# shanice-l/UNOPose

Hardware: AMD Instinct MI355X
Metric: (query,ref) pairs/sec forward (higher is better)
Workload: dtype bf16; 1 GPU; UNOPose.forward, batch 32 pairs/GPU, 2048 query pts, 5000->2048 reference pts, 196 coarse pts, 518x518 crops, DINOv2 ViT-B/14 reg4, random-init (trained-like) weights

## Files before the change

include/unopose_hip.h:

```cpp
#ifndef UNOPOSE_HIP_H
#define UNOPOSE_HIP_H

#include <stdint.h>

#ifdef __cplusplus
extern "C" {
#endif

#define UNOPOSE_OK 0
#define UNOPOSE_EINVAL 1
#define UNOPOSE_ELAUNCH 2
#define UNOPOSE_ENOMEM 3

typedef void *unopose_stream_t;

int unopose_abi_version(void);
const char *unopose_last_error(void);


int unopose_furthest_point_sampling(const float *xyz, int B, int N, int M,
                                    int32_t *idx, unopose_stream_t stream);

int unopose_gather_points(const float *points, const int32_t *idx, int B, int C,
                          int N, int M, float *out, unopose_stream_t stream);
// ... 110 lines not shown
int unopose_conv1x1_train_wgrad_blocks(void);
int unopose_conv1x1_train_forward(const float *x, int B, int cin, long L, const float *w, int cout, float *y, unopose_stream_t stream);
int unopose_conv1x1_train_wgrad(const float *dy, const float *x, int B, int cout, int cin, long L, float *workspace, float *dw,
                                unopose_stream_t stream);

int unopose_linear_wgrad_f32_splits(long rows, int N, int K);
int unopose_linear_wgrad_f32(const float *g, const float *x, long rows, int N, int K, float *workspace, float *dw, unopose_stream_t stream);

int unopose_linear_small_train_ws_floats(long rows, int N, int K);
int unopose_linear_small_train_forward(const float *x, const float *w, const float *bias, long rows, int N, int K, int relu, float *y,
                                       unopose_stream_t stream);
int unopose_linear_small_train_dx(const float *g, const float *y, const float *w, long rows, int N, int K, float *dx, unopose_stream_t stream);
int unopose_linear_small_train_dwdb(const float *g, const float *y, const float *x, long rows, int N, int K, float *workspace, long workspace_floats,
                                    float *dw, float *db, unopose_stream_t stream);
int unopose_linear_small_train_backward(const float *g, const float *y, const float *x, const float *w, long rows, int N, int K, float *workspace,
                                        long workspace_floats, float *dx, float *dw, float *db, unopose_stream_t stream);
int unopose_assign_labels(const float *atten, int B, int R, int C, const float *score1,
                          const float *score2, float *stats_ws, float *w1, float *w2,
                          unopose_stream_t stream);

int unopose_fine_correspondences(const float *atten, int B, int R, int C, const float *score1,
                                 const float *score2, const float *stats_ws, const float *w1,
                                 const float *w2, const float *pts2, float *weight, float *pred,
                                 unopose_stream_t stream);

int unopose_upproj_plan(const long long *choose, int B2, int Np, int H, int W, int side, int tok_offset, int tok_stride,
                        int cap_rows, int *ws, int *row_list, int *cellmap, int *tile_info, unopose_stream_t stream);

int unopose_linear_bf16_ld(const void *A, int lda, const void *W, int ldw, const float *bias, void *C, int ldc, long M, int N, int K,
                           int epilogue, unopose_stream_t stream);

int unopose_linear_add_layernorm_bf16(const void *A, const void *W, const float *bias, const void *resid, const float *ln_w,
                                      const float *ln_b, float eps, void *C, long M, int K, unopose_stream_t stream);

int unopose_linear_bf16_kv_vt(const void *A, const void *W, const float *bias, void *C, void *vt, long M, int N, int K, int tokens, int key_pad,
                              unopose_stream_t stream);

int unopose_linear_bf16_gather(const void *A, long M, int K, const void *W, int N, const float *bias, const int *row_list,
                               const int *tile_info, int max_tiles, void *C, unopose_stream_t stream);

int unopose_bilinear_sample_compact(const void *Cc, const int *cellmap, const long long *choose, int B2, int side, int Np,
                                    int H, int W, void *out, int out_bf16, unopose_stream_t stream);

int unopose_fine_assign(const void *f1, const void *f2, int B, int R, int C, int D, float shift, const float *score1,
                        const float *score2, const float *pts2, float *ws, float *w1, float *w2, float *weight,
                        float *pred, unopose_stream_t stream);

int unopose_min_dist(const float *p, const float *q, int B, int N, int M, const float *R,
                     const float *t, int cand_per_b, float *out, unopose_stream_t stream);

int unopose_coarse_hypotheses(const float *atten, int B, int R, int C, const float *score1,
                              const float *score2, const float *stats_ws, const float *w1,
                              const float *w2, const float *rand, int nprop, const float *pts1,
                              const float *pts2, float *cdf_ws, float *Rout, float *tout,
                              float *dis, unopose_stream_t stream);

int unopose_coarse_scores(const float *pts1, const float *pts2, int B, int n1, int n2,
                          const float *Rall, const float *tall, int nprop, const int64_t *top,
                          int ncand, const float *w1, float *score, unopose_stream_t stream);

int unopose_topk_smallest(const float *x, int B, int n, int k, int64_t *idx, unopose_stream_t stream);
int unopose_coarse_pick(const float *score, const int64_t *top, int B, int ncand, const float *Rall, const float *tall, int nprop,
                        float *R, float *t, float *best_score, unopose_stream_t stream);

int unopose_token_attention(const void *q, int ldq, const void *k, int ldk, const void *vt,
                            const void *qp, int ldqp, const void *E, int B, int n, int m,
// ... 215 lines not shown
```

unopose_amd/_lib.py:

```python
import ctypes
import os

import torch

_HERE = os.path.dirname(os.path.abspath(__file__))
SO_PATH = os.environ.get("UNOPOSE_LIB") or os.path.join(_HERE, "libunopose_hip.so")

_lib = None

_P = ctypes.c_void_p
_I = ctypes.c_int
_F = ctypes.c_float
_L = ctypes.c_long
_D = ctypes.c_double

SIGNATURES = {
    "unopose_furthest_point_sampling": [_P, _I, _I, _I, _P, _P],
    "unopose_gather_points": [_P, _P, _I, _I, _I, _I, _P, _P],
    "unopose_gather_points_grad": [_P, _P, _I, _I, _I, _I, _P, _P],
    "unopose_ball_query": [_P, _P, _I, _I, _I, _F, _I, _P, _P],
    "unopose_group_points": [_P, _P, _I, _I, _I, _I, _I, _P, _P],
    "unopose_group_points_grad": [_P, _P, _I, _I, _I, _I, _I, _P, _P],
    "unopose_three_nn": [_P, _P, _I, _I, _I, _P, _P, _P],
    "unopose_three_interpolate": [_P, _P, _P, _I, _I, _I, _I, _P, _P],
    "unopose_three_interpolate_grad": [_P, _P, _P, _I, _I, _I, _I, _P, _P],
    "unopose_lrf_global": [_P, _I, _I, _I, _P, _P],
    "unopose_query_lrf_group": [_P, _I, _I, _F, _I, _P, _P],
    "unopose_lrf_group_idx": [_P, _P, _P, _I, _I, _F, _I, _P, _P],
    "unopose_weighted_procrustes": [_P, _P, _P, _I, _I, _F, _F, _P, _P, _P],
    "unopose_assign_labels": [_P, _I, _I, _I, _P, _P, _P, _P, _P, _P],
    "unopose_linear_bf16_ld": [_P, _I, _P, _I, _P, _P, _I, ctypes.c_long, _I, _I, _I, _P],
    "unopose_scale_residual_layernorm_f32": [_P, _P, _P, _P, _P, ctypes.c_long, _I, _F, _P, _L, _P],
    "unopose_gather_rows": [_P, _I, _I, _I, _P, _I, _I, _I, _P, _L, _I, _P, _P],
    "unopose_softmax_stats": [_P, _I, _I, _I, _P, _P],
    "unopose_infonce_grad": [_P, _I, _I, _I, _P, _P, _P, _P, _P, _P],
    "unopose_fine_correspondences": [_P, _I, _I, _I, _P, _P, _P, _P, _P, _P, _P, _P, _P],
    "unopose_upproj_plan": [_P, _I, _I, _I, _I, _I, _I, _I, _I, _P, _P, _P, _P, _P],
    "unopose_linear_add_layernorm_bf16": [_P, _P, _P, _P, _P, _P, _F, _P, ctypes.c_long, _I, _P],
    "unopose_linear_bf16_kv_vt": [_P, _P, _P, _P, _P, ctypes.c_long, _I, _I, _I, _I, _P],
    "unopose_linear_bf16_gather": [_P, ctypes.c_long, _I, _P, _I, _P, _P, _P, _I, _P, _P],
    "unopose_bilinear_sample_compact": [_P, _P, _P, _I, _I, _I, _I, _I, _P, _I, _P],
    "unopose_fine_assign": [_P, _P, _I, _I, _I, _I, _F, _P, _P, _P, _P, _P, _P, _P, _P, _P],
    "unopose_min_dist": [_P, _P, _I, _I, _I, _P, _P, _I, _P, _P],
    "unopose_coarse_hypotheses": [_P, _I, _I, _I, _P, _P, _P, _P, _P, _P, _I, _P, _P, _P, _P, _P, _P, _P],
    "unopose_coarse_scores": [_P, _P, _I, _I, _I, _P, _P, _I, _P, _I, _P, _P, _P],
    "unopose_topk_smallest": [_P, _I, _I, _I, _P, _P],
    "unopose_coarse_pick": [_P, _P, _I, _I, _P, _P, _I, _P, _P, _P, _P],
    "unopose_token_attention": [_P, _I, _P, _I, _P, _P, _I, _P, _I, _I, _I, _F, _P, _P],
    "unopose_token_attention_key_pad": [],
    "unopose_token_attention_f32": [_P, _I, _P, _I, _P, _P, _I, _P, _I, _I, _I, _F, _P, _P],
    "unopose_token_attention_f32_train": [_P, _I, _P, _I, _P, _P, _I, _P, _I, _I, _I, _F, _P, _P, _P],
    "unopose_token_attention_f32_backward": [_P, _P, _I, _P, _I, _P, _P, _I, _P, _P, _I, _I, _I, _F, _P, _P, _P, _P, _P, _P, _P],
    "unopose_vit_attention_f32": [_P, _I, _I, _I, _P, _P],
    "unopose_vit_attention_f32_split": [_P, _I, _I, _I, _P, _P],
    "unopose_vit_attention_f32_ss": [_P, _I, _I, _I, _P, _P],
    "unopose_bn_train_chunk": [],
    "unopose_bn_relu_train_forward": [_P, _I, _I, ctypes.c_long, _P, _P, _F, _F, _P, _P, _P, _P, _P, _P, _P],
    "unopose_bn_relu_train_backward": [_P, _P, _I, _I, ctypes.c_long, _P, _P, _P, _P, _P, _P, _P, _P, _P],
    "unopose_bn_relu_maxpool_train_forward": [_P, _I, _I, _I, _I, _P, _P, _F, _F, _P, _P, _P, _P, _P, _P, _P, _P],
    "unopose_bn_relu_maxpool_train_backward": [_P, _P, _P, _I, _I, _I, _I, _P, _P, _P, _P, _P, _P, _P, _P, _P],
    "unopose_nearest_partner": [_P, _P, _I, _I, _I, _I, _F, _P, _P, _P, _P],
    "unopose_saliency_train_forward": [_P, _P, _P, _I, _I, _I, _P, _P, _P, _P, _P, _P, _P],
    "unopose_saliency_train_backward": [_P, _P, _P, _P, _P, _P, _P, _P, _P, _P, _P, _I, _I, _I, _P, _P, _P, _P],
    "unopose_match_train_pad": [],
    "unopose_match_train_split": [_P, _I, _I, _I, _I, _P, _P],
    "unopose_match_train_forward": [_P, _P, _I, _I, _I, _I, _I, _F, _P, _P, _P, _P, _P, _P, _P, _P],
    "unopose_match_train_backward": [_P, _P, _I, _I, _I, _I, _I, _F, _P, _P, _P, _P, _P, _P, _P, _P, _P, _P, _P, _P, _P, _P, _P, _P],
    "unopose_conv1x1_train_wgrad_blocks": [],
    "unopose_conv1x1_train_forward": [_P, _I, _I, ctypes.c_long, _P, _I, _P, _P],
    "unopose_conv1x1_train_wgrad": [_P, _P, _I, _I, _I, ctypes.c_long, _P, _P, _P],
    "unopose_linear_wgrad_f32_splits": [ctypes.c_long, _I, _I],
# ... 180 lines not shown
```

unopose_amd/build.py:

```python
import os
import subprocess
import sys
from concurrent.futures import ThreadPoolExecutor

HERE = os.path.dirname(os.path.abspath(__file__))
CSRC = os.path.join(HERE, "csrc")
OBJ = os.path.join(HERE, "csrc", "_obj")
SO = os.path.join(HERE, "libunopose_hip.so")
ARCH = "gfx950"
FLAGS = ["-O3", "-fno-slp-vectorize", "-fno-vectorize", "-std=c++17", "-fPIC", "-ffp-contract=off",
         f"--offload-arch={ARCH}", "-Wall", "-Wno-unused-function"]
EXTRA_FLAGS = {f: ["-fno-honor-nans"] for f in
               ("pe.hip", "embed.hip", "attn.hip", "attn_f32.hip", "vit_attn.hip", "vit_attn_f32s.hip", "linattn.hip", "bn_train.hip", "fused.hip", "gemm.hip", "gemm_small.hip", "fineassign.hip")}


def _hipcc():
    for c in (os.environ.get("HIPCC"), "/opt/rocm/bin/hipcc", "hipcc"):
        if c and (os.path.isabs(c) and os.path.exists(c) or not os.path.isabs(c)):
            return c
    raise RuntimeError("hipcc not found")


def _newer(src, dst, extra=()):
    if not os.path.exists(dst):
        return True
    t = os.path.getmtime(dst)
    return any(os.path.getmtime(p) > t for p in (src, *extra))


def build(force=False, verbose=False):
    os.makedirs(OBJ, exist_ok=True)
    hipcc = _hipcc()
    srcs = sorted(f for f in os.listdir(CSRC) if f.endswith(".hip"))
    hdrs = [os.path.join(CSRC, f) for f in os.listdir(CSRC) if f.endswith(".h")]
    hdrs.append(os.path.join(HERE, "..", "include", "unopose_hip.h"))
    jobs = []
    objs = []
    key = " ".join(FLAGS) + " | " + repr(sorted(EXTRA_FLAGS.items()))
    key_file = os.path.join(OBJ, "flags.txt")
    if not os.path.exists(key_file) or open(key_file).read() != key:
        force = True
    for f in srcs:
        src = os.path.join(CSRC, f)
        obj = os.path.join(OBJ, f[:-4] + ".o")
        objs.append(obj)
        if force or _newer(src, obj, hdrs + [os.path.abspath(__file__)]):
# ... 26 lines not shown
```

unopose_amd/model/modules.py:

```python
import math

import torch
import torch.nn as nn
import torch.nn.functional as F

from .. import ops


class _Attention(nn.Module):
    def __init__(self, dim, heads):
        super().__init__()
        self.heads = heads
        self.qkv = nn.Linear(dim, 3 * dim)
        self.proj = nn.Linear(dim, dim)

    def forward(self, x):
        B, T, C = x.shape
        qkv = ops.linear(x, self.qkv)
        o = ops.vit_attention(qkv, self.heads)
        return ops.linear(o, self.proj)


class _LayerScale(nn.Module):
    def __init__(self, dim):
# ... 302 lines not shown
        self.attention = _MHA(d, rpe)
        self.linear = nn.Linear(d, d)
        self.norm = nn.LayerNorm(d)


class _AttentionOutput(nn.Module):
    def __init__(self, d):
        super().__init__()
        self.expand = nn.Linear(d, 2 * d)
        self.squeeze = nn.Linear(2 * d, d)
        self.norm = nn.LayerNorm(d)

    def forward(self, x, out=None):
        if x.is_cuda and not ops.is_differentiable():
            return ops.ffn_add_layernorm(x, self.expand, self.squeeze, self.norm, out=out)
        assert out is None
        return ops.add_layernorm_train(x, ops.linear(ops.linear(x, self.expand, relu=True), self.squeeze), self.norm)


class TransformerLayer(nn.Module):

    def __init__(self, d, rpe, heads=4):
        super().__init__()
        self.heads = heads
        self.attention = _AttentionLayer(d, rpe)
        self.output = _AttentionOutput(d)

    def forward(self, x, mem, embed=None, out=None):
        a = self.attention
        if mem is None:
            mem = x
        h = ops.token_attention(x, mem, a.attention, self.heads, embed)
        if x.is_cuda and not ops.is_differentiable():
            x = ops.linear_add_layernorm(h, a.linear, x, a.norm)
        else:
            x = ops.add_layernorm_train(ops.linear(h, a.linear), x, a.norm)
        return self.output(x, out=out)


class GeometricTransformer(nn.Module):

    def __init__(self, d, heads=4):
        super().__init__()
        self.layers = nn.ModuleList([TransformerLayer(d, True, heads), TransformerLayer(d, False, heads)])

    def forward(self, f0, e0, f1, e1):
        e_all = _adjacent(e0, e1)
        if e_all is not None and f0.shape == f1.shape:
            f = _adjacent(f0, f1)
            f = self.forward_stacked(torch.cat([f0, f1], 0) if f is None else f, e_all)
            B = f0.shape[0]
            return f[:B], f[B:]
        f0 = self.layers[0](f0, f0, e0)
        f1 = self.layers[0](f1, f1, e1)
        f0 = self.layers[1](f0, f1)
        f1 = self.layers[1](f1, f0)
        return f0, f1

    def forward_stacked(self, f, e_all):
        B = f.shape[0] // 2
        f = self.layers[0](f, None, e_all)
        if ops.USE_STACKED_OUT and f.is_cuda and not ops.is_differentiable():
            out = torch.empty_like(f, memory_format=torch.contiguous_format)
            f0 = self.layers[1](f[:B], f[B:], out=out[:B])
            self.layers[1](f[B:], f0, out=out[B:])
            return out
        f0 = self.layers[1](f[:B], f[B:])
# ... 7 lines not shown
        return None
    return e0.as_strided((2 * e0.shape[0],) + tuple(e0.shape[1:]), e0.stride())


class _LinearAttention(nn.Module):
    def __init__(self, d):
        super().__init__()
        self.proj_q = nn.Linear(d, d)
        self.proj_k = nn.Linear(d, d)
        self.proj_v = nn.Linear(d, d)
        self.scale = nn.Parameter(torch.zeros(1, 1, d))


class _LinearAttentionLayer(nn.Module):
    def __init__(self, d):
        super().__init__()
        self.attention = _LinearAttention(d)
        self.linear = nn.Linear(d, d)
        self.norm = nn.LayerNorm(d)


class LinearTransformerLayer(nn.Module):

    def __init__(self, d, heads=4, focusing_factor=3):
        super().__init__()
        self.heads, self.focusing_factor = heads, focusing_factor
        self.attention = _LinearAttentionLayer(d)
        self.output = _AttentionOutput(d)

    def forward(self, x, mem, kv_skip=0):
        a = self.attention
        h = ops.focused_linear_attention(x, mem, a.attention, self.heads, self.focusing_factor, kv_skip=kv_skip)
        if x.is_cuda and not ops.is_differentiable():
            x = ops.linear_add_layernorm(h, a.linear, x, a.norm)
        else:
            x = ops.add_layernorm_train(ops.linear(h, a.linear), x, a.norm)
        return self.output(x)


class SparseToDenseTransformer(nn.Module):

    def __init__(self, d, heads=4, focusing_factor=3):
        super().__init__()
        self.sparse_layer = GeometricTransformer(d, heads)
        self.dense_layer = LinearTransformerLayer(d, heads, focusing_factor)

    @staticmethod
    def _sample(dense, fps_idx):
        return torch.cat([dense[:, 0:1], ops.gather_rows(dense, fps_idx)], dim=1)

    def forward(self, d0, e0, i0, d1, e1, i1):
        f0, f1 = self.sparse_layer(self._sample(d0, i0), e0, self._sample(d1, i1), e1)
        if d0.shape == d1.shape and f0.shape == f1.shape:
            B = d0.shape[0]
            nn_ = self.dense_layer(torch.cat([d0[:, 1:], d1[:, 1:]], 0), torch.cat([f0[:, 1:], f1[:, 1:]], 0))
            n0, n1 = nn_[:B], nn_[B:]
        else:
            n0 = self.dense_layer(d0[:, 1:], f0[:, 1:])
            n1 = self.dense_layer(d1[:, 1:], f1[:, 1:])
        return torch.cat([f0[:, 0:1], n0], 1), torch.cat([f1[:, 0:1], n1], 1)

    def forward_stacked(self, dense, bg, e_all, idx_all):
        f = self.sparse_layer.forward_stacked(ops.gather_rows(dense, idx_all, off=1, alt=bg, prepend=True), e_all)
        if not ops.USE_STACKED_OUT:
            return self.dense_layer(dense, f[:, 1:].contiguous()), f[:, 0:1].contiguous()
        return self.dense_layer(dense, f, kv_skip=1), f[:, 0:1]

# ... 113 lines not shown
```

unopose_amd/ops/__init__.py:

```python
import sys
import types

from . import _state
from .common import (
    _c, differentiable, is_differentiable, _fallbacks_seen, note_fallback, _params_key, _SPLIT_MEMO, _MUTATION_EPOCH, note_mutation,
    clear_split_memo, _aligned16, _no_autograd, _f32_path, _own_f32, _own_glue,
)
from .dense import (
    linear_backend, _bf16_weights, linear_bf16_hip, own_gemm_ok, bf16_linear_2d, f32x3_ok, split_f32, _f32x3_weights, linear_f32x3,
    linear_f32x3_bf16, linear_f32_raw, _transposed_weights, _LinearFn, _SmallLinearFn, small_linear_train_ok, _ZERO_BIAS, _zero_bias, linear_train, _lin, mlp, linear,
    ffn_add_layernorm, linear_add_layernorm, patch_embed, vit_prologue_ok, vit_prologue, vit_prologue_f32_ok, vit_prologue_f32, bmm_nt_f32, score_head, add_layernorm,
    _AddLayerNormFn, add_layernorm_train_ok, add_layernorm_train,
    scale_residual_, scale_residual_layernorm_f32_, vit_f32_fused_ok, scale_residual_layernorm_, ln_fold_ok, _fold_producer_weights,
    _fold_consumer_weights, linear_residual_, linear_lnfold, fold_shift, fold_row_means, _into,
)
from .attention import (
    vit_attention, vit_attention_f32_split, vit_attention_f32_ss, vit_attention_torch, _KEY_PAD, token_attention,
    _token_attention_hip_f32, _attn_weights, _token_attention_hip, token_attention_torch, _key_pad, _transpose_pad_f32, _TokenAttnFn,
    token_attention_train_ok, _token_attention_train, focused_linear_attention, _LinearAttnFn, linear_attention_train_ok,
    _focused_linear_attention_train, _la_workspace,
    _focused_linear_attention_hip_f32, _focused_linear_attention_hip, focused_linear_attention_torch,
)
from .geometry import (
    lrf_global, query_lrf_group, lrf_group_idx, weighted_procrustes, cloud_radius, scale_by_radius, gather_rows, pairwise_distance,
    _bf16_split, _mfma_fragment_order, _GEO_HINV, _GEO_D_RANGE, _GEO_TABLE_UNAVAILABLE, _geo_tables, geo_embedding, geo_embedding_torch,
    pe_group_mlp_max, pe_group_mlp_max_unfused, pe_geometry, pe_mlp_max, _pe_image, furthest_point_sample, _geo_grid, _GeoEmbedFn, geo_embedding_train_ok,
)
from .sampling import (
    bilinear_sample_native, sparse_upproj_ok, upproj_plan, sparse_pixel_features, bilinear_sample_pixels,
)
from .pose import (
    overlap_scores, set_first_rows_, pose_score, rigid_rows, feature_similarity, soft_assignment, coarse_pose_torch, fine_pose_torch, _assign_labels, _check_score_width,
    coarse_pose, fine_pose, fine_pose_fused_ok, normalize_rows_bf16, normalize_rows_f32, fine_pose_from_features,
)
from .prep import (
    PrepPlan, _desc_ints, _tap_table, prep_norm_table, _require, _result, prep_crop_resize, prep_lift, prep_gather,
)
from .augment import AugTables, color_augment, finish_crops
from .rle import pack_segs, rle_decode, rle_encode, window_masks
from .score import vsd_counts, pose_errors, pose_metrics, adi, gt_visibility, pts_extent, ref_select
from .vis import compose_poses
from .train import (
    _InfoNCEFn, infonce_two_way, _BNReLUTrain, bn_relu, _BNReLUMaxPoolTrain, bn_relu_maxpool, _SaliencyFn, saliency_pair,
    _match_split, _MatchHeadFn, _match_head_domain, match_head_train_ok, match_head, nearest_partner, _CONV_FWD_PAIRS, _CONV_WGRAD_PAIRS, _conv1x1_pair_ok, _conv1x1_wgrad_ok, _Conv1x1Fn, conv1x1,
# ... 26 lines not shown
```

unopose_amd/ops/dense.py:

```python
import ctypes

import torch
import torch.nn.functional as F

from .._lib import call, lib, on_device, ptr, stream_ptr
from . import _state as st
from .common import _MUTATION_EPOCH, _SPLIT_MEMO, _aligned16, _c, _f32_path, _no_autograd, _params_key, note_fallback, note_mutation


def linear_backend():
    if st.USE_HIP_GEMM and st.HIP_GEMM_ALL:
        return "csrc/gemm.hip (256x256x64 LDS-DMA tiles, persistent; bias / bias + erf-GELU epilogue) for every ViT linear"
    if st.USE_HIP_GEMM:
        return "hipBLASLt (through torch); fc1 + GELU: csrc/gemm.hip (256x256x64 LDS-DMA tiles, fused bias + erf-GELU epilogue)"
    return "hipBLASLt (through torch)"


def _bf16_weights(lin):
    key = _params_key(lin)
    cache = getattr(lin, "_bf16_cache", None)
    if cache is None or cache[0] != key:
        with torch.no_grad():
            b32 = torch.zeros(lin.weight.shape[0], device=lin.weight.device) if lin.bias is None else lin.bias.detach().float().contiguous()
            cache = (key, lin.weight.detach().to(torch.bfloat16).contiguous(),
# ... 312 lines not shown
def _into(out, y):
    if out is None:
        return y
    note_mutation()
    out.copy_(y)
    return out


def linear_add_layernorm(h, lin, x, norm, out=None):
    N, K = lin.weight.shape
    rows = h.numel() // K
    if (st.USE_FUSED_LINEAR_LN and not st._DIFF and h.is_cuda and torch.is_autocast_enabled() and st.HIP_GEMM_ALL and N == 256
            and own_gemm_ok(rows, N, K) and tuple(norm.normalized_shape) == (256,) and norm.weight is not None and norm.bias is not None and lin.bias is not None):
        cache = _bf16_weights(lin)
        with torch.autocast("cuda", enabled=False):
            hb = _c(h if h.dtype == torch.bfloat16 else h.to(torch.bfloat16)).reshape(rows, K)
            xb = _c(x if x.dtype == torch.bfloat16 else x.to(torch.bfloat16)).reshape(rows, N)
            direct = out is not None and out.dtype == torch.bfloat16 and out.is_contiguous() and out.numel() == rows * N and out.device == h.device
            if direct:
                note_mutation()
            y = out if direct else torch.empty(rows, N, dtype=torch.bfloat16, device=h.device)
            with on_device(h.device):
                call("unopose_linear_add_layernorm_bf16", ptr(hb), ptr(cache[1]), ptr(cache[3]), ptr(xb), ptr(norm.weight.detach()),
                     ptr(norm.bias.detach()), float(norm.eps), ptr(y), rows, K, stream_ptr())
        return out if direct else _into(out, y.reshape(*h.shape[:-1], N))
    if out is not None and h.is_cuda and not st._DIFF and out.shape == x.shape and out.is_contiguous() and out.dtype in (torch.float32, torch.bfloat16):
        y = linear(h, lin)
        if y.dtype in (torch.float32, torch.bfloat16) and (out.dtype == (torch.bfloat16 if torch.is_autocast_enabled() else y.dtype)):
            return add_layernorm(y, x, norm, out=out)
        return _into(out, add_layernorm(y, x, norm))
    return _into(out, add_layernorm(linear(h, lin), x, norm))


def patch_embed(patches, conv):
    w = conv.weight.reshape(conv.weight.shape[0], -1)
    D, K = w.shape
    rows = patches.numel() // K
    if _f32_path(patches) and f32x3_ok(rows, D, 32):
        Kp = (K + 31) // 32 * 32
        key = _params_key(conv, Kp, "f32")
        cache = getattr(conv, "_f32x3_pad_cache", None)
        if cache is None or cache[0] != key:
            with torch.no_grad():
                wp = torch.zeros(D, Kp, dtype=torch.float32, device=w.device)
                wp[:, :K] = w.detach()
                b = torch.zeros(D, device=w.device) if conv.bias is None else conv.bias.detach().float().contiguous()
                cache = (key, split_f32(wp), b)
            conv._f32x3_pad_cache = cache
        a = torch.zeros(rows, Kp, dtype=torch.float32, device=patches.device)
        a[:, :K] = patches.reshape(rows, K)
        return linear_f32x3(split_f32(a), cache[1], cache[2], rows, D, Kp).reshape(*patches.shape[:-1], D)
    if st._DIFF or not (st.HIP_GEMM_ALL and patches.is_cuda and torch.is_autocast_enabled() and own_gemm_ok(rows, D, 64)):
        return F.linear(patches, w, conv.bias)
    Kp = (K + 63) // 64 * 64
    key = _params_key(conv, Kp)
    cache = getattr(conv, "_bf16_pad_cache", None)
    if cache is None or cache[0] != key:
        with torch.no_grad():
            wp = torch.zeros(D, Kp, dtype=torch.bfloat16, device=w.device)
            wp[:, :K] = w.detach()
            b = torch.zeros(D, device=w.device) if conv.bias is None else conv.bias.detach().float().contiguous()
        cache = (key, wp, b)
        conv._bf16_pad_cache = cache
    with torch.autocast("cuda", enabled=False):
        a = torch.zeros(rows, Kp, dtype=torch.bfloat16, device=patches.device)
        a[:, :K] = patches.reshape(rows, K)
# ... 358 lines not shown
```

Before: 1116 pairs/s.

## Fuse attention output linear, add-LayerNorm and FFN into one layer-tail kernel

Adds a persistent HIP kernel that, for each 64- or 128-row tile, computes the attention output projection with residual add and LayerNorm, then the 256->512->256 ReLU FFN with a second residual add and LayerNorm. The intermediates stay in LDS and registers. Geometric transformer layers call it instead of separate linear_add_layernorm and ffn_add_layernorm launches. The aim is to remove the global-memory round trips of the intermediate activations and the extra kernel launches. In exchange, each block loads all three weight matrices through a double-buffered ring, occupancy is one block per CU with large LDS, and the kernel only applies to 256/512 dimensions.

```diff
diff --git a/include/unopose_hip.h b/include/unopose_hip.h
--- a/include/unopose_hip.h
+++ b/include/unopose_hip.h
@@ -166,6 +166,11 @@
 
 int unopose_linear_add_layernorm_bf16(const void *A, const void *W, const float *bias, const void *resid, const float *ln_w,
                                       const float *ln_b, float eps, void *C, long M, int K, unopose_stream_t stream);
+
+int unopose_layer_tail_rows64_max(void);
+int unopose_layer_tail_bf16(const void *h, const void *x, const void *Wl, const float *bl, const float *lna_w, const float *lna_b,
+                            float eps_a, const void *W1, const float *b1, const void *W2, const float *b2, const float *lno_w,
+                            const float *lno_b, float eps_o, void *y, long rows, unopose_stream_t stream);
 
 int unopose_linear_bf16_kv_vt(const void *A, const void *W, const float *bias, void *C, void *vt, long M, int N, int K, int tokens, int key_pad,
                               unopose_stream_t stream);
diff --git a/unopose_amd/_lib.py b/unopose_amd/_lib.py
--- a/unopose_amd/_lib.py
+++ b/unopose_amd/_lib.py
@@ -37,6 +37,8 @@
     "unopose_fine_correspondences": [_P, _I, _I, _I, _P, _P, _P, _P, _P, _P, _P, _P, _P],
     "unopose_upproj_plan": [_P, _I, _I, _I, _I, _I, _I, _I, _I, _P, _P, _P, _P, _P],
     "unopose_linear_add_layernorm_bf16": [_P, _P, _P, _P, _P, _P, _F, _P, ctypes.c_long, _I, _P],
+    "unopose_layer_tail_rows64_max": [],
+    "unopose_layer_tail_bf16": [_P, _P, _P, _P, _P, _P, _F, _P, _P, _P, _P, _P, _P, _F, _P, _L, _P],
     "unopose_linear_bf16_kv_vt": [_P, _P, _P, _P, _P, ctypes.c_long, _I, _I, _I, _I, _P],
     "unopose_linear_bf16_gather": [_P, ctypes.c_long, _I, _P, _I, _P, _P, _P, _I, _P, _P],
     "unopose_bilinear_sample_compact": [_P, _P, _P, _I, _I, _I, _I, _I, _P, _I, _P],
diff --git a/unopose_amd/build.py b/unopose_amd/build.py
--- a/unopose_amd/build.py
+++ b/unopose_amd/build.py
@@ -11,7 +11,7 @@
 FLAGS = ["-O3", "-fno-slp-vectorize", "-fno-vectorize", "-std=c++17", "-fPIC", "-ffp-contract=off",
          f"--offload-arch={ARCH}", "-Wall", "-Wno-unused-function"]
 EXTRA_FLAGS = {f: ["-fno-honor-nans"] for f in
-               ("pe.hip", "embed.hip", "attn.hip", "attn_f32.hip", "vit_attn.hip", "vit_attn_f32s.hip", "linattn.hip", "bn_train.hip", "fused.hip", "gemm.hip", "gemm_small.hip", "fineassign.hip")}
+               ("pe.hip", "embed.hip", "attn.hip", "attn_f32.hip", "vit_attn.hip", "vit_attn_f32s.hip", "linattn.hip", "bn_train.hip", "fused.hip", "gemm.hip", "gemm_small.hip", "layer_tail.hip", "fineassign.hip")}
 
 
 def _hipcc():
diff --git a/unopose_amd/csrc/layer_tail.hip b/unopose_amd/csrc/layer_tail.hip
--- /dev/null
+++ b/unopose_amd/csrc/layer_tail.hip
@@ -0,0 +1,549 @@
+#include "gemm_common.h"
+
+namespace unopose {
+
+#define LT_RING 0
+#define LT_HY 65536
+#define LT_E 98304
+#define LT_STAT 131072
+#define LT_LDS_BYTES (131072 + 64 * 4 * 8)
+
+struct LayerTailArgs {
+  const u16 *h, *x, *Wl, *W1, *W2;
+  const float *bl, *b1, *b2, *lna_w, *lna_b, *lno_w, *lno_b;
+  float eps_a, eps_o;
+  u16 *y;
+  int rows, tiles;
+};
+
+__global__ __launch_bounds__(256, 1) void layer_tail_kernel(const LayerTailArgs p) {
+  extern __shared__ __attribute__((aligned(1024))) char smem[];
+  const int tid = threadIdx.x, lane = tid & 63, wave = __builtin_amdgcn_readfirstlane(tid >> 6);
+  const int wn = wave;
+  const int l31 = lane & 31, hi = lane >> 5;
+  const int per_xcd = (p.tiles + 7) >> 3;
+  const int t_id = (blockIdx.x & 7) * per_xcd + (blockIdx.x >> 3);
+  if (t_id >= p.tiles) return;
+  const int M = p.rows, m0 = t_id * 64;
+  const __amdgpu_buffer_rsrc_t h_rs = __builtin_amdgcn_make_buffer_rsrc((void *)p.h, 0, (int)((size_t)M * 512), 0x00020000);
+  const __amdgpu_buffer_rsrc_t x_rs = __builtin_amdgcn_make_buffer_rsrc((void *)p.x, 0, (int)((size_t)M * 512), 0x00020000);
+  const __amdgpu_buffer_rsrc_t y_rs = __builtin_amdgcn_make_buffer_rsrc((void *)p.y, 0, (int)((size_t)M * 512), 0x00020000);
+  const __amdgpu_buffer_rsrc_t wl_rs = __builtin_amdgcn_make_buffer_rsrc((void *)p.Wl, 0, 256 * 256 * 2, 0x00020000);
+  const __amdgpu_buffer_rsrc_t w1_rs = __builtin_amdgcn_make_buffer_rsrc((void *)p.W1, 0, 512 * 256 * 2, 0x00020000);
+  const __amdgpu_buffer_rsrc_t w2_rs = __builtin_amdgcn_make_buffer_rsrc((void *)p.W2, 0, 256 * 512 * 2, 0x00020000);
+  const uint32_t lds0 = (uint32_t)(uintptr_t)(__attribute__((address_space(3))) char *)smem;
+
+  const int r8 = lane >> 3;
+  const int c_sw = (lane & 7) ^ (((wave & 1) << 2) | (r8 >> 1));
+  const uint32_t lane256 = (uint32_t)((r8 * 256 + c_sw * 8) * 2);
+  const uint32_t lane512 = (uint32_t)((r8 * 512 + c_sw * 8) * 2);
+  auto issue = [&](int ps, int t, int buf) {
+    const uint32_t dst = lds0 + LT_RING + buf * 32768;
+#pragma unroll
+    for (int i = 0; i < 8; ++i) {
+      const int j = wave + 4 * i;
+      if (ps == 0)
+        gemm_dma16(dst + j * 1024, lane256 + (uint32_t)(j * 8 * 512), wl_rs, t * 128);
+      else if (ps == 1 || ps == 3)
+        gemm_dma16(dst + j * 1024, lane256 + (uint32_t)(((ps == 3 ? 256 : 0) + j * 8) * 512), w1_rs, t * 128);
+      else
+        gemm_dma16(dst + j * 1024, lane512 + (uint32_t)(j * 8 * 1024), w2_rs, ((ps == 4 ? 4 : 0) + t) * 128);
+    }
+  };
+  const int fx = (l31 >> 1) & 7;
+  uint32_t fr_off[4];
+#pragma unroll
+  for (int ks = 0; ks < 4; ++ks) fr_off[ks] = (uint32_t)((l31 >> 3) * 1024 + (l31 & 7) * 128 + ((((ks << 1) | hi) ^ fx) << 4));
+  const uint32_t w_base = (uint32_t)(wn * 64 * 128);
+
+#pragma unroll
+  for (int t = 0; t < 4; ++t)
+#pragma unroll
+    for (int i = 0; i < 2; ++i) {
+      const int j = wave + 4 * i;
+      gemm_dma16(lds0 + LT_HY + t * 8192 + j * 1024, lane256 + (uint32_t)(m0 + j * 8) * 512u, h_rs, t * 128);
+    }
+#pragma unroll
+  for (int t = 0; t < 4; ++t)
+#pragma unroll
+    for (int i = 0; i < 2; ++i) {
+      const int j = wave + 4 * i;
+      gemm_dma16(lds0 + LT_E + t * 8192 + j * 1024, lane256 + (uint32_t)(m0 + j * 8) * 512u, x_rs, t * 128);
+    }
+  issue(0, 0, 0);
+
+  int s = 0;
+  auto pass = [&](const char *aimg, f32x16(&acc)[2][2]) {
+#pragma unroll
+    for (int t = 0; t < 4; ++t) {
+      if (s + 1 < 20) {
+        issue((s + 1) >> 2, (s + 1) & 3, (s + 1) & 1);
+        asm volatile("s_waitcnt vmcnt(8)" ::: "memory");
+      } else {
+        asm volatile("s_waitcnt vmcnt(0)" ::: "memory");
+      }
+      __builtin_amdgcn_s_barrier();
+      asm volatile("" ::: "memory");
+      const char *wb = smem + LT_RING + (s & 1) * 32768 + w_base;
+      const char *ab = aimg + t * 8192;
+      bf16x8 wf[2][2], af[2][2];
+#pragma unroll
+      for (int nb = 0; nb < 2; ++nb) wf[0][nb] = *reinterpret_cast<const bf16x8 *>(wb + nb * 4096 + fr_off[0]);
+#pragma unroll
+      for (int mb = 0; mb < 2; ++mb) af[0][mb] = *reinterpret_cast<const bf16x8 *>(ab + mb * 4096 + fr_off[0]);
+#pragma unroll
+      for (int ks = 0; ks < 4; ++ks) {
+        if (ks + 1 < 4) {
+#pragma unroll
+          for (int nb = 0; nb < 2; ++nb) wf[(ks + 1) & 1][nb] = *reinterpret_cast<const bf16x8 *>(wb + nb * 4096 + fr_off[ks + 1]);
+#pragma unroll
+          for (int mb = 0; mb < 2; ++mb) af[(ks + 1) & 1][mb] = *reinterpret_cast<const bf16x8 *>(ab + mb * 4096 + fr_off[ks + 1]);
+          __builtin_amdgcn_sched_barrier(0);
+        }
+#pragma unroll
+        for (int nb = 0; nb < 2; ++nb)
+#pragma unroll
+          for (int mb = 0; mb < 2; ++mb) acc[nb][mb] = __builtin_amdgcn_mfma_f32_32x32x16_bf16(wf[ks & 1][nb], af[ks & 1][mb], acc[nb][mb], 0, 0, 0);
+      }
+      asm volatile("s_waitcnt lgkmcnt(0)" ::: "memory");
+      __builtin_amdgcn_s_barrier();
+      asm volatile("" ::: "memory");
+      ++s;
+    }
+  };
+  auto zero = [&](f32x16(&acc)[2][2]) {
+#pragma unroll
+    for (int nb = 0; nb < 2; ++nb)
+#pragma unroll
+      for (int mb = 0; mb < 2; ++mb)
+#pragma unroll
+        for (int r = 0; r < 16; ++r) acc[nb][mb][r] = 0.f;
+  };
+  auto load_bias = [&](const float *b, float4(&bv)[2][4]) {
+#pragma unroll
+    for (int nb = 0; nb < 2; ++nb)
+#pragma unroll
+      for (int g = 0; g < 4; ++g) bv[nb][g] = *reinterpret_cast<const float4 *>(b + wn * 64 + nb * 32 + 8 * g + 4 * hi);
+  };
+  auto img_off = [&](int mb, int nb, int g) {
+    const int row = mb * 32 + l31;
+    return wn * 8192 + row * 128 + (((4 * nb + g) ^ ((row >> 1) & 7)) << 4) + 8 * hi;
+  };
+  float2 *ln_part = reinterpret_cast<float2 *>(smem + LT_STAT);
+  auto layernorm = [&](f32x16(&acc)[2][2], const float(&a1)[2], const float(&a2)[2], const float *ln_w, const float *ln_b, float ln_eps) {
+#pragma unroll
+    for (int mb = 0; mb < 2; ++mb) {
+      float s1 = a1[mb], s2 = a2[mb];
+      s1 += __shfl_xor(s1, 32);
+      s2 += __shfl_xor(s2, 32);
+      if (hi == 0) ln_part[(mb * 32 + l31) * 4 + wn] = make_float2(s1, s2);
+    }
+    __syncthreads();
+#pragma unroll
+    for (int mb = 0; mb < 2; ++mb) {
+      const float2 *pp = ln_part + (mb * 32 + l31) * 4;
+      const float t1 = (pp[0].x + pp[1].x) + (pp[2].x + pp[3].x), t2 = (pp[0].y + pp[1].y) + (pp[2].y + pp[3].y);
+      const float mean = t1 * (1.f / 256);
+      const float rstd = rsqrtf(fmaxf(t2 * (1.f / 256) - mean * mean, 0.f) + ln_eps);
+#pragma unroll
+      for (int nb = 0; nb < 2; ++nb)
+#pragma unroll
+        for (int g = 0; g < 4; ++g) {
+          const int nl = wn * 64 + nb * 32 + 8 * g + 4 * hi;
+          const float4 gw = *reinterpret_cast<const float4 *>(ln_w + nl), gb = *reinterpret_cast<const float4 *>(ln_b + nl);
+          acc[nb][mb][4 * g + 0] = (acc[nb][mb][4 * g + 0] - mean) * rstd * gw.x + gb.x;
+          acc[nb][mb][4 * g + 1] = (acc[nb][mb][4 * g + 1] - mean) * rstd * gw.y + gb.y;
+          acc[nb][mb][4 * g + 2] = (acc[nb][mb][4 * g + 2] - mean) * rstd * gw.z + gb.z;
+          acc[nb][mb][4 * g + 3] = (acc[nb][mb][4 * g + 3] - mean) * rstd * gw.w + gb.w;
+        }
+    }
+  };
+
+  f32x16 acc[2][2], acc3[2][2];
+  float4 bv[2][4];
+  float a1[2], a2[2];
+
+  load_bias(p.bl, bv);
+  zero(acc);
+  pass(smem + LT_HY, acc);
+#pragma unroll
+  for (int mb = 0; mb < 2; ++mb) {
+    float s1 = 0.f, s2 = 0.f;
+#pragma unroll
+    for (int nb = 0; nb < 2; ++nb)
+#pragma unroll
+      for (int g = 0; g < 4; ++g) {
+        const uint2 r = *reinterpret_cast<const uint2 *>(smem + LT_E + img_off(mb, nb, g));
+        const float v0 = acc[nb][mb][4 * g + 0] + bv[nb][g].x + __uint_as_float(r.x << 16);
+        const float v1 = acc[nb][mb][4 * g + 1] + bv[nb][g].y + __uint_as_float(r.x & 0xffff0000u);
+        const float v2 = acc[nb][mb][4 * g + 2] + bv[nb][g].z + __uint_as_float(r.y << 16);
+        const float v3 = acc[nb][mb][4 * g + 3] + bv[nb][g].w + __uint_as_float(r.y & 0xffff0000u);
+        acc[nb][mb][4 * g + 0] = v0;
+        acc[nb][mb][4 * g + 1] = v1;
+        acc[nb][mb][4 * g + 2] = v2;
+        acc[nb][mb][4 * g + 3] = v3;
+        s1 += (v0 + v1) + (v2 + v3);
+        s2 += (v0 * v0 + v1 * v1) + (v2 * v2 + v3 * v3);
+      }
+    a1[mb] = s1;
+    a2[mb] = s2;
+  }
+  layernorm(acc, a1, a2, p.lna_w, p.lna_b, p.eps_a);
+#pragma unroll
+  for (int mb = 0; mb < 2; ++mb)
+#pragma unroll
+    for (int nb = 0; nb < 2; ++nb)
+#pragma unroll
+      for (int g = 0; g < 4; ++g)
+        *reinterpret_cast<uint2 *>(smem + LT_HY + img_off(mb, nb, g)) =
+            make_uint2(cvt_pk_bf16_f32(acc[nb][mb][4 * g + 0], acc[nb][mb][4 * g + 1]), cvt_pk_bf16_f32(acc[nb][mb][4 * g + 2], acc[nb][mb][4 * g + 3]));
+  __syncthreads();
+
+  zero(acc3);
+#pragma unroll
+  for (int c = 0; c < 2; ++c) {
+    load_bias(p.b1 + 256 * c, bv);
+    zero(acc);
+    pass(smem + LT_HY, acc);
+#pragma unroll
+    for (int mb = 0; mb < 2; ++mb)
+#pragma unroll
+      for (int nb = 0; nb < 2; ++nb)
+#pragma unroll
+        for (int g = 0; g < 4; ++g) {
+          const float v0 = fmaxf(acc[nb][mb][4 * g + 0] + bv[nb][g].x, 0.f), v1 = fmaxf(acc[nb][mb][4 * g + 1] + bv[nb][g].y, 0.f);
+          const float v2 = fmaxf(acc[nb][mb][4 * g + 2] + bv[nb][g].z, 0.f), v3 = fmaxf(acc[nb][mb][4 * g + 3] + bv[nb][g].w, 0.f);
+          *reinterpret_cast<uint2 *>(smem + LT_E + img_off(mb, nb, g)) = make_uint2(cvt_pk_bf16_f32(v0, v1), cvt_pk_bf16_f32(v2, v3));
+        }
+    __syncthreads();
+    if (c == 1) load_bias(p.b2, bv);
+    pass(smem + LT_E, acc3);
+  }
+
+#pragma unroll
+  for (int mb = 0; mb < 2; ++mb) {
+    float s1 = 0.f, s2 = 0.f;
+#pragma unroll
+    for (int nb = 0; nb < 2; ++nb)
+#pragma unroll
+      for (int g = 0; g < 4; ++g) {
+        const uint2 r = *reinterpret_cast<const uint2 *>(smem + LT_HY + img_off(mb, nb, g));
+        const float v0 = acc3[nb][mb][4 * g + 0] + bv[nb][g].x + __uint_as_float(r.x << 16);
+        const float v1 = acc3[nb][mb][4 * g + 1] + bv[nb][g].y + __uint_as_float(r.x & 0xffff0000u);
+        const float v2 = acc3[nb][mb][4 * g + 2] + bv[nb][g].z + __uint_as_float(r.y << 16);
+        const float v3 = acc3[nb][mb][4 * g + 3] + bv[nb][g].w + __uint_as_float(r.y & 0xffff0000u);
+        acc3[nb][mb][4 * g + 0] = v0;
+        acc3[nb][mb][4 * g + 1] = v1;
+        acc3[nb][mb][4 * g + 2] = v2;
+        acc3[nb][mb][4 * g + 3] = v3;
+        s1 += (v0 + v1) + (v2 + v3);
+        s2 += (v0 * v0 + v1 * v1) + (v2 * v2 + v3 * v3);
+      }
+    a1[mb] = s1;
+    a2[mb] = s2;
+  }
+  layernorm(acc3, a1, a2, p.lno_w, p.lno_b, p.eps_o);
+  char *cw = smem + LT_RING + wave * 8192;
+#pragma unroll
+  for (int mb = 0; mb < 2; ++mb)
+#pragma unroll
+    for (int nb = 0; nb < 2; ++nb)
+#pragma unroll
+      for (int g = 0; g < 4; ++g) {
+        const int nl = nb * 32 + 8 * g + 4 * hi;
+        const int row = mb * 32 + l31;
+        const int slot16 = (nl >> 3) ^ (row & 7);
+        *reinterpret_cast<uint2 *>(cw + row * 128 + slot16 * 16 + (nl & 4) * 2) =
+            make_uint2(cvt_pk_bf16_f32(acc3[nb][mb][4 * g + 0], acc3[nb][mb][4 * g + 1]), cvt_pk_bf16_f32(acc3[nb][mb][4 * g + 2], acc3[nb][mb][4 * g + 3]));
+      }
+  __builtin_amdgcn_fence(__ATOMIC_RELEASE, "wavefront");
+  __builtin_amdgcn_wave_barrier();
+  __builtin_amdgcn_fence(__ATOMIC_ACQUIRE, "wavefront");
+  const uint32_t c_v0 = (uint32_t)((((size_t)m0 + (lane >> 3)) * 256 + wn * 64 + (lane & 7) * 8) * 2);
+#pragma unroll
+  for (int it = 0; it < 8; ++it) {
+    const int row = it * 8 + (lane >> 3), q = lane & 7;
+    const u32x4 v = *reinterpret_cast<const u32x4 *>(cw + row * 128 + ((q ^ (row & 7)) << 4));
+    __builtin_amdgcn_raw_buffer_store_b128(v, y_rs, c_v0 + (uint32_t)(it * 8 * 512), 0, 0);
+  }
+}
+
+#define LT2_Y1 65536
+#define LT2_EQ 131072
+#define LT2_LDS_BYTES 163840
+
+template <int NB>
+__device__ __forceinline__ void lt2_ktile(const char *wb, const char *ab, const uint32_t (&fr_off)[4], f32x16 (&acc)[NB][4]) {
+  bf16x8 wf[2][NB], af[2][4];
+#pragma unroll
+  for (int nb = 0; nb < NB; ++nb) wf[0][nb] = *reinterpret_cast<const bf16x8 *>(wb + nb * 4096 + fr_off[0]);
+#pragma unroll
+  for (int mb = 0; mb < 4; ++mb) af[0][mb] = *reinterpret_cast<const bf16x8 *>(ab + mb * 4096 + fr_off[0]);
+#pragma unroll
+  for (int ks = 0; ks < 4; ++ks) {
+    if (ks + 1 < 4) {
+#pragma unroll
+      for (int nb = 0; nb < NB; ++nb) wf[(ks + 1) & 1][nb] = *reinterpret_cast<const bf16x8 *>(wb + nb * 4096 + fr_off[ks + 1]);
+#pragma unroll
+      for (int mb = 0; mb < 4; ++mb) af[(ks + 1) & 1][mb] = *reinterpret_cast<const bf16x8 *>(ab + mb * 4096 + fr_off[ks + 1]);
+      __builtin_amdgcn_sched_barrier(0);
+    }
+#pragma unroll
+    for (int nb = 0; nb < NB; ++nb)
+#pragma unroll
+      for (int mb = 0; mb < 4; ++mb) acc[nb][mb] = __builtin_amdgcn_mfma_f32_32x32x16_bf16(wf[ks & 1][nb], af[ks & 1][mb], acc[nb][mb], 0, 0, 0);
+  }
+}
+
+__global__ __launch_bounds__(256, 1) void layer_tail128_kernel(const LayerTailArgs p) {
+  extern __shared__ __attribute__((aligned(1024))) char smem[];
+  const int tid = threadIdx.x, lane = tid & 63, wave = __builtin_amdgcn_readfirstlane(tid >> 6);
+  const int wn = wave;
+  const int l31 = lane & 31, hi = lane >> 5;
+  const int per_xcd = (p.tiles + 7) >> 3;
+  const int t_id = (blockIdx.x & 7) * per_xcd + (blockIdx.x >> 3);
+  if (t_id >= p.tiles) return;
+  const int M = p.rows, m0 = t_id * 128;
+  const __amdgpu_buffer_rsrc_t h_rs = __builtin_amdgcn_make_buffer_rsrc((void *)p.h, 0, (int)((size_t)M * 512), 0x00020000);
+  const __amdgpu_buffer_rsrc_t y_rs = __builtin_amdgcn_make_buffer_rsrc((void *)p.y, 0, (int)((size_t)M * 512), 0x00020000);
+  const __amdgpu_buffer_rsrc_t wl_rs = __builtin_amdgcn_make_buffer_rsrc((void *)p.Wl, 0, 256 * 256 * 2, 0x00020000);
+  const __amdgpu_buffer_rsrc_t w1_rs = __builtin_amdgcn_make_buffer_rsrc((void *)p.W1, 0, 512 * 256 * 2, 0x00020000);
+  const __amdgpu_buffer_rsrc_t w2_rs = __builtin_amdgcn_make_buffer_rsrc((void *)p.W2, 0, 256 * 512 * 2, 0x00020000);
+  const uint32_t lds0 = (uint32_t)(uintptr_t)(__attribute__((address_space(3))) char *)smem;
+  const int r8 = lane >> 3;
+  const int c_sw = (lane & 7) ^ (((wave & 1) << 2) | (r8 >> 1));
+  const uint32_t lane256 = (uint32_t)((r8 * 256 + c_sw * 8) * 2);
+  const uint32_t lane512 = (uint32_t)((r8 * 512 + c_sw * 8) * 2);
+  auto pieces = [](int s) { return (s < 4 || (s - 4) % 6 >= 4) ? 8 : 4; };
+  auto issue = [&](int s, int buf) {
+    const uint32_t dst = lds0 + LT_RING + buf * 32768;
+    const int q = (s - 4) / 6, r = (s - 4) % 6;
+#pragma unroll
+    for (int i = 0; i < 8; ++i) {
+      const int j = wave + 4 * i;
+      if (s < 4)
+        gemm_dma16(dst + j * 1024, lane256 + (uint32_t)(j * 8 * 512), wl_rs, s * 128);
+      else if (r >= 4)
+        gemm_dma16(dst + j * 1024, lane512 + (uint32_t)(j * 8 * 1024), w2_rs, (2 * q + r - 4) * 128);
+      else if (i < 4)
+        gemm_dma16(dst + j * 1024, lane256 + (uint32_t)((128 * q + j * 8) * 512), w1_rs, r * 128);
+    }
+  };
+  const int fx = (l31 >> 1) & 7;
+  uint32_t fr_off[4];
+#pragma unroll
+  for (int ks = 0; ks < 4; ++ks) fr_off[ks] = (uint32_t)((l31 >> 3) * 1024 + (l31 & 7) * 128 + ((((ks << 1) | hi) ^ fx) << 4));
+
+#pragma unroll
+  for (int t = 0; t < 4; ++t)
+#pragma unroll
+    for (int i = 0; i < 4; ++i) {
+      const int j = wave + 4 * i;
+      gemm_dma16(lds0 + LT2_Y1 + t * 16384 + j * 1024, lane256 + (uint32_t)(m0 + j * 8) * 512u, h_rs, t * 128);
+    }
+  issue(0, 0);
+
+  int buf = 0, s = 0;
+  auto tile_begin = [&]() {
+    if (s + 1 < 28) {
+      issue(s + 1, buf ^ 1);
+      if (pieces(s + 1) == 8)
+        asm volatile("s_waitcnt vmcnt(8)" ::: "memory");
+      else
+        asm volatile("s_waitcnt vmcnt(4)" ::: "memory");
+    } else {
+      asm volatile("s_waitcnt vmcnt(0)" ::: "memory");
+    }
+    __builtin_amdgcn_s_barrier();
+    asm volatile("" ::: "memory");
+  };
+  auto tile_end = [&]() {
+    asm volatile("s_waitcnt lgkmcnt(0)" ::: "memory");
+    __builtin_amdgcn_s_barrier();
+    asm volatile("" ::: "memory");
+    buf ^= 1;
+    ++s;
+  };
+  auto img_off = [&](int mb, int nb, int g) {
+    const int row = mb * 32 + l31;
+    return wn * 16384 + row * 128 + (((4 * nb + g) ^ ((row >> 1) & 7)) << 4) + 8 * hi;
+  };
+  auto load_bias = [&](const float *b, float4(&bv)[2][4]) {
+#pragma unroll
+    for (int nb = 0; nb < 2; ++nb)
+#pragma unroll
+      for (int g = 0; g < 4; ++g) bv[nb][g] = *reinterpret_cast<const float4 *>(b + wn * 64 + nb * 32 + 8 * g + 4 * hi);
+  };
+  float2 *ln_part = reinterpret_cast<float2 *>(smem + LT2_EQ);
+  auto add_layernorm = [&](f32x16(&acc)[2][4], const float4(&bv)[2][4], auto resid, const float *ln_w, const float *ln_b, float ln_eps) {
+#pragma unroll
+    for (int mb = 0; mb < 4; ++mb) {
+      float a1 = 0.f, a2 = 0.f;
+#pragma unroll
+      for (int nb = 0; nb < 2; ++nb)
+#pragma unroll
+        for (int g = 0; g < 4; ++g) {
+          const uint2 r = resid(mb, nb, g);
+          const float v0 = acc[nb][mb][4 * g + 0] + bv[nb][g].x + __uint_as_float(r.x << 16);
+          const float v1 = acc[nb][mb][4 * g + 1] + bv[nb][g].y + __uint_as_float(r.x & 0xffff0000u);
+          const float v2 = acc[nb][mb][4 * g + 2] + bv[nb][g].z + __uint_as_float(r.y << 16);
+          const float v3 = acc[nb][mb][4 * g + 3] + bv[nb][g].w + __uint_as_float(r.y & 0xffff0000u);
+          acc[nb][mb][4 * g + 0] = v0;
+          acc[nb][mb][4 * g + 1] = v1;
+          acc[nb][mb][4 * g + 2] = v2;
+          acc[nb][mb][4 * g + 3] = v3;
+          a1 += (v0 + v1) + (v2 + v3);
+          a2 += (v0 * v0 + v1 * v1) + (v2 * v2 + v3 * v3);
+        }
+      a1 += __shfl_xor(a1, 32);
+      a2 += __shfl_xor(a2, 32);
+      if (hi == 0) ln_part[(mb * 32 + l31) * 4 + wn] = make_float2(a1, a2);
+    }
+    __syncthreads();
+#pragma unroll
+    for (int mb = 0; mb < 4; ++mb) {
+      const float2 *pp = ln_part + (mb * 32 + l31) * 4;
+      const float t1 = (pp[0].x + pp[1].x) + (pp[2].x + pp[3].x), t2 = (pp[0].y + pp[1].y) + (pp[2].y + pp[3].y);
+      const float mean = t1 * (1.f / 256);
+      const float rstd = rsqrtf(fmaxf(t2 * (1.f / 256) - mean * mean, 0.f) + ln_eps);
+#pragma unroll
+      for (int nb = 0; nb < 2; ++nb)
+#pragma unroll
+        for (int g = 0; g < 4; ++g) {
+          const int nl = wn * 64 + nb * 32 + 8 * g + 4 * hi;
+          const float4 gw = *reinterpret_cast<const float4 *>(ln_w + nl), gb = *reinterpret_cast<const float4 *>(ln_b + nl);
+          acc[nb][mb][4 * g + 0] = (acc[nb][mb][4 * g + 0] - mean) * rstd * gw.x + gb.x;
+          acc[nb][mb][4 * g + 1] = (acc[nb][mb][4 * g + 1] - mean) * rstd * gw.y + gb.y;
+          acc[nb][mb][4 * g + 2] = (acc[nb][mb][4 * g + 2] - mean) * rstd * gw.z + gb.z;
+          acc[nb][mb][4 * g + 3] = (acc[nb][mb][4 * g + 3] - mean) * rstd * gw.w + gb.w;
+        }
+    }
+    __syncthreads();
+  };
+
+  f32x16 acc[2][4], acc3[2][4];
+  float4 bv[2][4];
+  load_bias(p.bl, bv);
+#pragma unroll
+  for (int nb = 0; nb < 2; ++nb)
+#pragma unroll
+    for (int mb = 0; mb < 4; ++mb)
+#pragma unroll
+      for (int r = 0; r < 16; ++r) acc[nb][mb][r] = 0.f, acc3[nb][mb][r] = 0.f;
+#pragma unroll
+  for (int t = 0; t < 4; ++t) {
+    tile_begin();
+    lt2_ktile<2>(smem + LT_RING + buf * 32768 + wn * 8192, smem + LT2_Y1 + t * 16384, fr_off, acc);
+    tile_end();
+  }
+  add_layernorm(
+      acc, bv,
+      [&](int mb, int nb, int g) {
+        const int m = min(m0 + mb * 32 + l31, M - 1);
+        return *reinterpret_cast<const uint2 *>(p.x + (size_t)m * 256 + wn * 64 + 4 * hi + nb * 32 + 8 * g);
+      },
+      p.lna_w, p.lna_b, p.eps_a);
+#pragma unroll
+  for (int mb = 0; mb < 4; ++mb)
+#pragma unroll
+    for (int nb = 0; nb < 2; ++nb)
+#pragma unroll
+      for (int g = 0; g < 4; ++g)
+        *reinterpret_cast<uint2 *>(smem + LT2_Y1 + img_off(mb, nb, g)) =
+            make_uint2(cvt_pk_bf16_f32(acc[nb][mb][4 * g + 0], acc[nb][mb][4 * g + 1]), cvt_pk_bf16_f32(acc[nb][mb][4 * g + 2], acc[nb][mb][4 * g + 3]));
+  __syncthreads();
+
+#pragma unroll
+  for (int q = 0; q < 4; ++q) {
+    float4 b1v[4];
+#pragma unroll
+    for (int g = 0; g < 4; ++g) b1v[g] = *reinterpret_cast<const float4 *>(p.b1 + 128 * q + wn * 32 + 8 * g + 4 * hi);
+    f32x16 acc2[1][4];
+#pragma unroll
+    for (int mb = 0; mb < 4; ++mb)
+#pragma unroll
+      for (int r = 0; r < 16; ++r) acc2[0][mb][r] = 0.f;
+#pragma unroll
+    for (int t = 0; t < 4; ++t) {
+      tile_begin();
+      lt2_ktile<1>(smem + LT_RING + buf * 32768 + wn * 4096, smem + LT2_Y1 + t * 16384, fr_off, acc2);
+      tile_end();
+    }
+#pragma unroll
+    for (int mb = 0; mb < 4; ++mb)
+#pragma unroll
+      for (int g = 0; g < 4; ++g) {
+        const float v0 = fmaxf(acc2[0][mb][4 * g + 0] + b1v[g].x, 0.f), v1 = fmaxf(acc2[0][mb][4 * g + 1] + b1v[g].y, 0.f);
+        const float v2 = fmaxf(acc2[0][mb][4 * g + 2] + b1v[g].z, 0.f), v3 = fmaxf(acc2[0][mb][4 * g + 3] + b1v[g].w, 0.f);
+        const int row = mb * 32 + l31;
+        *reinterpret_cast<uint2 *>(smem + LT2_EQ + (wn >> 1) * 16384 + row * 128 + (((4 * (wn & 1) + g) ^ ((row >> 1) & 7)) << 4) + 8 * hi) =
+            make_uint2(cvt_pk_bf16_f32(v0, v1), cvt_pk_bf16_f32(v2, v3));
+      }
+    __syncthreads();
+#pragma unroll
+    for (int t = 0; t < 2; ++t) {
+      tile_begin();
+      lt2_ktile<2>(smem + LT_RING + buf * 32768 + wn * 8192, smem + LT2_EQ + t * 16384, fr_off, acc3);
+      tile_end();
+    }
+  }
+
+  load_bias(p.b2, bv);
+  add_layernorm(
+      acc3, bv, [&](int mb, int nb, int g) { return *reinterpret_cast<const uint2 *>(smem + LT2_Y1 + img_off(mb, nb, g)); }, p.lno_w, p.lno_b,
+      p.eps_o);
+  char *cw = smem + LT_RING + wave * 16384;
+#pragma unroll
+  for (int mb = 0; mb < 4; ++mb)
+#pragma unroll
+    for (int nb = 0; nb < 2; ++nb)
+#pragma unroll
+      for (int g = 0; g < 4; ++g) {
+        const int nl = nb * 32 + 8 * g + 4 * hi;
+        const int row = mb * 32 + l31;
+        const int slot16 = (nl >> 3) ^ (row & 7);
+        *reinterpret_cast<uint2 *>(cw + row * 128 + slot16 * 16 + (nl & 4) * 2) =
+            make_uint2(cvt_pk_bf16_f32(acc3[nb][mb][4 * g + 0], acc3[nb][mb][4 * g + 1]), cvt_pk_bf16_f32(acc3[nb][mb][4 * g + 2], acc3[nb][mb][4 * g + 3]));
+      }
+  __builtin_amdgcn_fence(__ATOMIC_RELEASE, "wavefront");
+  __builtin_amdgcn_wave_barrier();
+  __builtin_amdgcn_fence(__ATOMIC_ACQUIRE, "wavefront");
+  const uint32_t c_v0 = (uint32_t)((((size_t)m0 + (lane >> 3)) * 256 + wn * 64 + (lane & 7) * 8) * 2);
+#pragma unroll
+  for (int it = 0; it < 16; ++it) {
+    const int row = it * 8 + (lane >> 3), q = lane & 7;
+    const u32x4 v = *reinterpret_cast<const u32x4 *>(cw + row * 128 + ((q ^ (row & 7)) << 4));
+    __builtin_amdgcn_raw_buffer_store_b128(v, y_rs, c_v0 + (uint32_t)(it * 8 * 512), 0, 0);
+  }
+}
+
+}
+
+using namespace unopose;
+
+extern "C" int unopose_layer_tail_rows64_max(void) { return 64 * gemm_cu_count(); }
+
+extern "C" int unopose_layer_tail_bf16(const void *h, const void *x, const void *Wl, const float *bl, const float *lna_w, const float *lna_b,
+                                       float eps_a, const void *W1, const float *b1, const void *W2, const float *b2, const float *lno_w,
+                                       const float *lno_b, float eps_o, void *y, long rows, unopose_stream_t stream) {
+  UNOPOSE_REQUIRE(h && x && Wl && bl && lna_w && lna_b && W1 && b1 && W2 && b2 && lno_w && lno_b && y, "layer_tail_bf16: null pointer");
+  UNOPOSE_REQUIRE(rows >= 1 && rows < (1L << 22), "layer_tail_bf16: needs 1 <= rows < 2^22 (got %ld)", rows);
+  static bool opt[64] = {false}, opt2[64] = {false};
+  if (lds_optin(opt, (const void *)layer_tail_kernel, LT_LDS_BYTES, "layer_tail_bf16") != UNOPOSE_OK ||
+      lds_optin(opt2, (const void *)layer_tail128_kernel, LT2_LDS_BYTES, "layer_tail_bf16") != UNOPOSE_OK)
+    return UNOPOSE_ELAUNCH;
+  LayerTailArgs a;
+  a.h = (const u16 *)h, a.x = (const u16 *)x, a.Wl = (const u16 *)Wl, a.W1 = (const u16 *)W1, a.W2 = (const u16 *)W2;
+  a.bl = bl, a.b1 = b1, a.b2 = b2, a.lna_w = lna_w, a.lna_b = lna_b, a.lno_w = lno_w, a.lno_b = lno_b;
+  a.eps_a = eps_a, a.eps_o = eps_o;
+  a.y = (u16 *)y;
+  a.rows = (int)rows;
+  if (rows <= unopose_layer_tail_rows64_max()) {
+    a.tiles = cdiv(rows, 64);
+    hipLaunchKernelGGL(layer_tail_kernel, dim3(((a.tiles + 7) >> 3) << 3), dim3(256), LT_LDS_BYTES, (hipStream_t)stream, a);
+  } else {
+    a.tiles = cdiv(rows, 128);
+    hipLaunchKernelGGL(layer_tail128_kernel, dim3(((a.tiles + 7) >> 3) << 3), dim3(256), LT2_LDS_BYTES, (hipStream_t)stream, a);
+  }
+  return check_launch("layer_tail_bf16");
+}
diff --git a/unopose_amd/model/modules.py b/unopose_amd/model/modules.py
--- a/unopose_amd/model/modules.py
+++ b/unopose_amd/model/modules.py
@@ -358,7 +358,8 @@
             mem = x
         h = ops.token_attention(x, mem, a.attention, self.heads, embed)
         if x.is_cuda and not ops.is_differentiable():
-            x = ops.linear_add_layernorm(h, a.linear, x, a.norm)
+            o = self.output
+            return ops.layer_tail(h, a.linear, x, a.norm, o.expand, o.squeeze, o.norm, out=out)
         else:
             x = ops.add_layernorm_train(ops.linear(h, a.linear), x, a.norm)
         return self.output(x, out=out)
@@ -432,7 +433,8 @@
         a = self.attention
         h = ops.focused_linear_attention(x, mem, a.attention, self.heads, self.focusing_factor, kv_skip=kv_skip)
         if x.is_cuda and not ops.is_differentiable():
-            x = ops.linear_add_layernorm(h, a.linear, x, a.norm)
+            o = self.output
+            return ops.layer_tail(h, a.linear, x, a.norm, o.expand, o.squeeze, o.norm)
         else:
             x = ops.add_layernorm_train(ops.linear(h, a.linear), x, a.norm)
         return self.output(x)
diff --git a/unopose_amd/ops/__init__.py b/unopose_amd/ops/__init__.py
--- a/unopose_amd/ops/__init__.py
+++ b/unopose_amd/ops/__init__.py
@@ -9,7 +9,7 @@
 from .dense import (
     linear_backend, _bf16_weights, linear_bf16_hip, own_gemm_ok, bf16_linear_2d, f32x3_ok, split_f32, _f32x3_weights, linear_f32x3,
     linear_f32x3_bf16, linear_f32_raw, _transposed_weights, _LinearFn, _SmallLinearFn, small_linear_train_ok, _ZERO_BIAS, _zero_bias, linear_train, _lin, mlp, linear,
-    ffn_add_layernorm, linear_add_layernorm, patch_embed, vit_prologue_ok, vit_prologue, vit_prologue_f32_ok, vit_prologue_f32, bmm_nt_f32, score_head, add_layernorm,
+    ffn_add_layernorm, linear_add_layernorm, _layer_tail_ok, layer_tail, patch_embed, vit_prologue_ok, vit_prologue, vit_prologue_f32_ok, vit_prologue_f32, bmm_nt_f32, score_head, add_layernorm,
     _AddLayerNormFn, add_layernorm_train_ok, add_layernorm_train,
     scale_residual_, scale_residual_layernorm_f32_, vit_f32_fused_ok, scale_residual_layernorm_, ln_fold_ok, _fold_producer_weights,
     _fold_consumer_weights, linear_residual_, linear_lnfold, fold_shift, fold_row_means, _into,
diff --git a/unopose_amd/ops/dense.py b/unopose_amd/ops/dense.py
--- a/unopose_amd/ops/dense.py
+++ b/unopose_amd/ops/dense.py
@@ -368,6 +368,36 @@
     return _into(out, add_layernorm(linear(h, lin), x, norm))
 
 
+def _layer_tail_ok(h, lin, x, norm_a, expand, squeeze, norm_o):
+    if not (h.is_cuda and torch.is_autocast_enabled() and not st._DIFF and st.HIP_GEMM_ALL and st.USE_HIP_GEMM and st.USE_FUSED_LINEAR_LN):
+        return False
+    if tuple(lin.weight.shape) != (256, 256) or tuple(expand.weight.shape) != (512, 256) or tuple(squeeze.weight.shape) != (256, 512):
+        return False
+    if h.shape[-1] != 256 or x.shape != h.shape or not 1 <= h.numel() // 256 < 2 ** 22:
+        return False
+    return (all(tuple(n.normalized_shape) == (256,) and n.weight is not None and n.bias is not None for n in (norm_a, norm_o))
+            and all(l.bias is not None for l in (lin, expand, squeeze)))
+
+
+def layer_tail(h, lin, x, norm_a, expand, squeeze, norm_o, out=None):
+    if not _layer_tail_ok(h, lin, x, norm_a, expand, squeeze, norm_o):
+        return ffn_add_layernorm(linear_add_layernorm(h, lin, x, norm_a), expand, squeeze, norm_o, out=out)
+    rows = h.numel() // 256
+    cl, c1, c2 = _bf16_weights(lin), _bf16_weights(expand), _bf16_weights(squeeze)
+    with torch.autocast("cuda", enabled=False):
+        hb = _c(h if h.dtype == torch.bfloat16 else h.to(torch.bfloat16))
+        xb = _c(x if x.dtype == torch.bfloat16 else x.to(torch.bfloat16))
+        direct = out is not None and out.dtype == torch.bfloat16 and out.is_contiguous() and out.numel() == rows * 256 and out.device == h.device
+        if direct:
+            note_mutation()
+        y = out if direct else torch.empty(rows, 256, dtype=torch.bfloat16, device=h.device)
+        with on_device(h.device):
+            call("unopose_layer_tail_bf16", ptr(hb), ptr(xb), ptr(cl[1]), ptr(cl[3]), ptr(norm_a.weight.detach()), ptr(norm_a.bias.detach()),
+                 float(norm_a.eps), ptr(c1[1]), ptr(c1[3]), ptr(c2[1]), ptr(c2[3]), ptr(norm_o.weight.detach()), ptr(norm_o.bias.detach()),
+                 float(norm_o.eps), ptr(y), rows, stream_ptr())
+    return out if direct else _into(out, y.reshape(h.shape))
+
+
 def patch_embed(patches, conv):
     w = conv.weight.reshape(conv.weight.shape[0], -1)
     D, K = w.shape
```

After: 1123 pairs/s, median of 6. About the same (+0.6%).
